# frobelbest/BANet

Hardware: NVIDIA H100
Metric: LM iters/sec (frame-pair LM iterations, 640x480x4-scale, K=128) (higher is better)
Workload: dtype tf32 level-wise (mma.sync tf32 x3 below 65536 points/pair, x1 above; f32 accumulate; everything else f32)

## Files before the change

### banet_b200/csrc/lm_build_tc6.cu

```cuda
#include "common.cuh"
#include "features.cuh"
#include "lm_build.h"
#include "tc_utils.cuh"
#include "mma_role.cuh"
#include "tmap.h"
#include <stdlib.h>

namespace banet { namespace v6 {
using namespace tc;

constexpr int TILE = 64, W0 = 4, GW = 8, AW = 4, MW = 4;
constexpr int THREADS = (W0 + GW + AW + MW) * 32;
constexpr int STAGE_A = 4 * TILE * 128, STAGE_R = 5 * TILE * 128;
constexpr int REC = 16;

template <int MODE, bool FLY, bool BB = false> struct Smem {
#ifndef BANET_TC6_NST1
#define BANET_TC6_NST1 4
#endif
#ifndef BANET_TC6_NST2
#define BANET_TC6_NST2 3
#endif
#ifndef BANET_TC6_NST3
#define BANET_TC6_NST3 2
#endif
#ifndef BANET_TC6_NREC
#define BANET_TC6_NREC 3
#endif
    static constexpr int NST = MODE == 1 ? BANET_TC6_NST1 : MODE == 2 ? BANET_TC6_NST2 : BANET_TC6_NST3;
    static constexpr int NREC = MODE == 3 ? 2 : BANET_TC6_NREC;
    static constexpr int STAGE = BB ? STAGE_A / 2 : STAGE_A;
    static constexpr int off_A = 0;
    static constexpr int off_R = NST * STAGE;
    static constexpr int off_Alo = off_R + STAGE_R;
    static constexpr int off_Rlo = off_Alo + (MODE >= 2 && !BB ? STAGE_A : 0);
    static constexpr int off_misc = off_Rlo + (MODE == 3 ? STAGE_R : 0);
    static constexpr int off_bar = off_misc;
    static constexpr int off_tile = off_misc + 192;
    static constexpr int off_pose = off_tile + 64;
    static constexpr int off_w = off_pose + W0 * 16 * 4;
    static constexpr int off_rec = off_w + W0 * 128 * 4;
    static constexpr int off_rbs = off_rec + NREC * TILE * REC * 4;
    static constexpr int off_ccs = off_rbs + GW * 128 * 4;
    static constexpr int total = off_ccs + AW * 28 * 4;
    static constexpr int slack = 1024;
    static constexpr int bytes = total + slack;
};

__device__ __forceinline__ long long gtime6() { long long t; asm volatile("mov.u64 %0, %%globaltimer;" : "=l"(t)); return t; }
#ifdef BANET_TC6_TRACE_ON
#define TC6_TRACE(role, it, slot) do { if (prm.trace && blockIdx.x == 1 && lane == 0 && (it) >= 16 && (it) < 48) \
        prm.trace[(((role) * 32 + ((it) - 16)) * 12) + (slot)] = gtime6(); } while (0)
#else
#define TC6_TRACE(role, it, slot) do { } while (0)
#endif
template <int NT> __device__ __forceinline__ void team_bar() { asm volatile("bar.sync 2, %0;" :: "n"(NT) : "memory"); }
__device__ __forceinline__ int reflect_i(int i, int n) { i = i < 0 ? -i : (i >= n ? 2 * n - 2 - i : i); return i < 0 ? 0 : i; }
__device__ __forceinline__ float4 ldg4(const float* p) { return __ldg(reinterpret_cast<const float4*>(p)); }
__device__ __forceinline__ float hsum16(float v) {
    v += __shfl_xor_sync(0xffffffffu, v, 8); v += __shfl_xor_sync(0xffffffffu, v, 4);
    v += __shfl_xor_sync(0xffffffffu, v, 2); v += __shfl_xor_sync(0xffffffffu, v, 1);
    return v;
}
struct TileCoord { int b, n0, cnt, tx0, ty0; };
__device__ __forceinline__ TileCoord tile_coord(const BuildParams& prm, long long tl) {
    TileCoord tc;
    const unsigned t = (unsigned)tl, tpp = (unsigned)prm.tiles_per_pair;
    tc.b = (int)(t / tpp);
    const int r = (int)(t - (unsigned)tc.b * tpp);
    if (prm.grid_w > 0) {
// ... 37 lines not shown
template <int NCH, bool FLY, int NREC>
__device__ __forceinline__ void gather_bf16(const BuildParams& prm, const int* sTile, float* sRec, float* sRbs, uint64_t* recs, uint64_t* gath,
                                            uint64_t* rbdump, uint64_t* rbfree, int ntiles, int g, int lane)
{
    constexpr int C = 64 * NCH, CPL = C / 16, PXW = TILE / GW;
    using TB = BfTap<CPL>;
    const int hw = lane >> 4, hl = lane & 15;
    const int N = prm.N, h = prm.h, w = prm.w, c2 = prm.c2;
    float rb[CPL];
#pragma unroll
    for (int u = 0; u < CPL; ++u) rb[u] = 0.f;
    typename TB::T tb[13];
    int cur_b = -1, ndump = 0;
    const uint64_t pol_stream = prm.l2_hints >= 1 ? l2_policy_evict_first() : l2_policy_evict_normal();
    const uint64_t pol_tap = prm.l2_hints >= 2 ? l2_policy_evict_last() : l2_policy_evict_normal();

    auto dump_rb = [&]() {
        if (ndump > 0) mbar_wait_parked(rbfree, (ndump - 1) & 1);
#pragma unroll
        for (int u = 0; u < CPL; ++u) rb[u] += __shfl_xor_sync(0xffffffffu, rb[u], 16);
        if (hw == 0) {
#pragma unroll
            for (int j = 0; j < CPL / 4; ++j)
                *reinterpret_cast<float4*>(sRbs + g * 128 + CPL * hl + 4 * j) = make_float4(rb[4 * j], rb[4 * j + 1], rb[4 * j + 2], rb[4 * j + 3]);
        }
        __syncwarp();
        if (lane == 0) mbar_arrive(rbdump);
#pragma unroll
        for (int u = 0; u < CPL; ++u) rb[u] = 0.f;
        ++ndump;
    };

    for (int j = 0; j < ntiles; ++j) {
        const int s = j % NREC;
        mbar_wait_parked(&recs[s], (j / NREC) & 1);
        const int b = sTile[s * 4];
        if (b != cur_b) { if (cur_b >= 0) dump_rb(); cur_b = b; }
        float* rec = sRec + (s * TILE + g * PXW) * REC;
        const bf16* c1b = static_cast<const bf16*>(prm.conv1) + (size_t)b * N * C + CPL * hl;
        const bf16* img = static_cast<const bf16*>(prm.conv2) + (size_t)b * h * w * c2 + CPL * hl;
#pragma unroll
        for (int u = 0; u < PXW / 2; ++u) {
            const int pl = 2 * u + hw;
            const float mask = rec[pl * REC + 4];
            float m11 = 0.f, m12 = 0.f, m22 = 0.f, q1 = 0.f, q2 = 0.f;
            if (mask != 0.f) {
                const uint4 o = *reinterpret_cast<const uint4*>(rec + pl * REC);
                const int n = __float_as_int(rec[pl * REC + 11]);
                auto ldt = [&](const bf16* q) { return TB::ld(q, pol_tap); };
                tb[0] = TB::ld_stream(c1b + (size_t)n * C, pol_stream);
// ... 34 lines not shown
                    q1 = fmaf(gx, d, q1); q2 = fmaf(gy, d, q2);
                    rb[i] += fabsf(d);
                }
            }
            m11 = hsum16(m11); m12 = hsum16(m12); m22 = hsum16(m22); q1 = hsum16(q1); q2 = hsum16(q2);
            if (hl == 0) {
                const float wn = (prm.weight && mask != 0.f) ? __ldg(prm.weight + (size_t)b * N + __float_as_int(rec[pl * REC + 11])) : 1.f;
                *reinterpret_cast<float4*>(rec + pl * REC + 12) = make_float4(m11 * wn, m12 * wn, m22 * wn, q1 * wn);
                rec[pl * REC + 11] = q2 * wn;
            }
        }
        __syncwarp();
        if (lane == 0) mbar_arrive(&gath[s]);
    }
    if (cur_b >= 0) dump_rb();
}

template <int NCH, bool FLY, int MODE, int KBLK = 4, typename TF = float, typename TB = float>
__global__ void __launch_bounds__(THREADS, 1)
lm_build_tc6_kernel(const __grid_constant__ CUtensorMap tmapB, const BuildParams prm)
{
    constexpr bool BB = sizeof(TB) == 2;
    using SM = Smem<MODE, FLY, BB>;
    constexpr int NST = SM::NST, NREC = SM::NREC;
    constexpr int BLK = BB ? 4096 : 8192;
    constexpr int KR = 32 * KBLK, EXTB = KBLK;
    extern __shared__ __align__(1024) unsigned char smem_raw[];
    unsigned char* base = smem_raw + ((1024u - (smem_u32(smem_raw) & 1023u)) & 1023u);
    uint64_t* bars = reinterpret_cast<uint64_t*>(base + SM::off_bar);
    uint64_t* fullB = bars;
// ... 24 lines not shown
        for (int i = 0; i < NREC; ++i) { mbar_init(&recs[i], W0); mbar_init(&gath[i], GW); mbar_init(&recfree[i], AW); }
        mbar_init(rfree, MW); mbar_init(rready, AW);
        mbar_init(rbdump, GW); mbar_init(rbfree, AW);
        fence_barrier_init();
        prefetch_tmap(&tmapB);
    }
    for (int i = tid; i < TILE * 8; i += THREADS) {
        const int r = i >> 3, c = i & 7;
        *reinterpret_cast<float4*>(base + SM::off_R + EXTB * 8192 + sw128_off(r, c)) = make_float4(0.f, 0.f, 0.f, 0.f);
        if (MODE == 3) *reinterpret_cast<float4*>(base + SM::off_Rlo + EXTB * 8192 + sw128_off(r, c)) = make_float4(0.f, 0.f, 0.f, 0.f);
    }
    __syncthreads();

    const int r16 = lane & 15, hf = lane >> 4;

    if (warp < W0) {
        setmaxnreg_dec<48>();
        const int gwi = warp, nlr = gwi * 16 + r16;
        float* myPose = sPose + gwi * 16;
        float* myW = sW + gwi * 128;
        int geom_b = -1;
        uint32_t dseed = 0;
        TileCoord nxt = tile_coord(prm, t_begin);
        int nxt_r = (int)((unsigned)t_begin - (unsigned)nxt.b * (unsigned)prm.tiles_per_pair);
        for (int j = 0; j < ntiles; ++j) {
            const TileCoord tc = nxt;
            if (++nxt_r == prm.tiles_per_pair) { nxt_r = 0; ++nxt.b; nxt.tx0 = 0; nxt.ty0 = 0; nxt.n0 = 0; nxt.cnt = grid2d ? TILE : min(TILE, N); }
            else if (grid2d && prm.band_rows > 1) nxt = tile_coord(prm, t_begin + j + 1);
            else if (grid2d) { nxt.tx0 += 8; if (nxt.tx0 >= prm.tiles_x * 8) { nxt.tx0 = 0; nxt.ty0 += 8; } }
            else { nxt.n0 += TILE; nxt.cnt = min(TILE, N - nxt.n0); }
            const int b = tc.b;
            if (gwi == 1 && j + 2 < ntiles) {
                const TileCoord tn = tile_coord(prm, t_begin + j + 2);
                if (grid2d) {
                    if (lane < 8) {
                        const int gy = tn.ty0 + lane;
                        if (gy < prm.grid_h && tn.tx0 < prm.grid_w) {
                            const size_t n = (size_t)gy * prm.grid_w + tn.tx0;
                            const int wpx = min(8, prm.grid_w - tn.tx0);
// ... 28 lines not shown
                    dseed = (__float_as_uint(__ldg(prm.W + (size_t)b * KR)) * 0x9E3779B1u) ^ (__float_as_uint(__ldg(prm.W + (size_t)b * KR + 1)) * 0x85EBCA77u)
                          ^ (__float_as_uint(__ldg(prm.W + (size_t)b * KR + 2)) * 0xC2B2AE3Du) ^ __float_as_uint(__ldg(prm.T + b * 3)) ^ (uint32_t)b;
                __syncwarp();
            }
            const int s = j % NST, sr = j % NREC;
            const unsigned char* As = base + SM::off_A + s * SM::STAGE;
            float p0 = 0.f, p1 = 0.f, p2 = 0.f, D0 = 0.f;
            int n = 0; bool valid = false;
            if (grid2d) { const int gx = tc.tx0 + (nlr & 7), gy = tc.ty0 + (nlr >> 3); valid = gx < prm.grid_w && gy < prm.grid_h; n = gy * prm.grid_w + gx; }
            else { valid = nlr < tc.cnt; n = tc.n0 + nlr; }
            if (lane < 16 && valid) {
                const float* pp = prm.p + (size_t)b * 3 * N + n;
                p0 = __ldg(pp); p1 = __ldg(pp + N); p2 = __ldg(pp + 2 * (size_t)N);
                D0 = __ldg(prm.D + (size_t)b * N + n);
            }
            if (gwi == 0) TC6_TRACE(2, j, 0);
            mbar_wait_parked(&recfree[sr], ((j / NREC) & 1) ^ 1);
            mbar_wait_parked(&fullB[s], (j / NST) & 1);
            if (gwi == 0) TC6_TRACE(2, j, 1);
            float mydot;
            {
                float4 acc = make_float4(0.f, 0.f, 0.f, 0.f);
                uint4 bq = make_uint4(0u, 0u, 0u, 0u);
#pragma unroll
                for (int i = 0; i < 16; ++i) {
                    const int blk = 2 * hf + (i >> 3), c = i & 7;
                    if (KBLK != 4 && blk >= KBLK) continue;
                    float4 bv;
                    if constexpr (BB) {
                        if ((c & 1) == 0) bq = *reinterpret_cast<const uint4*>(As + blk * BLK + sw64_off(nlr, c >> 1));
                        const uint32_t u0 = (c & 1) ? bq.z : bq.x, u1 = (c & 1) ? bq.w : bq.y;
                        bv = make_float4(bf16_lo(u0), bf16_hi(u0), bf16_lo(u1), bf16_hi(u1));
                    } else {
                        bv = *reinterpret_cast<const float4*>(As + blk * 8192 + sw128_off(nlr, c));
// ... 3 lines not shown
                    if constexpr (MODE == 1 && !BB) {
                        uint32_t hsh = dseed ^ ((uint32_t)n * 0x9E3779B1u) ^ ((uint32_t)(blk * 8 + c) * 0x85EBCA77u);
                        hsh ^= hsh >> 16; hsh *= 0x7FEB352Du; hsh ^= hsh >> 15;
                        uint32_t hs2 = hsh * 0x846CA68Bu; hs2 ^= hs2 >> 16;
                        *reinterpret_cast<float4*>(const_cast<unsigned char*>(As) + blk * 8192 + sw128_off(nlr, c)) =
                            make_float4(__uint_as_float((__float_as_uint(bv.x) + (hsh & 0x1fffu)) & 0xFFFFE000u),
                                        __uint_as_float((__float_as_uint(bv.y) + ((hsh >> 13) & 0x1fffu)) & 0xFFFFE000u),
                                        __uint_as_float((__float_as_uint(bv.z) + (hs2 & 0x1fffu)) & 0xFFFFE000u),
                                        __uint_as_float((__float_as_uint(bv.w) + ((hs2 >> 13) & 0x1fffu)) & 0xFFFFE000u));
                    }
                }
                if constexpr (MODE == 1 && !BB) fence_proxy_async_smem();
                mydot = (acc.x + acc.y) + (acc.z + acc.w);
                mydot += __shfl_xor_sync(0xffffffffu, mydot, 16);
            }
            if (gwi == 0) TC6_TRACE(2, j, 2);
            if (lane < 16) {
                const float* pose = myPose;
                float mask = 0.f, x = 0.f, y = 0.f, iZ = 0.f, rx = 0.f, ry = 0.f, rz = 0.f, dx = 0.f, dy = 0.f;
                int x0 = 0, y0 = 0;
                if (valid) {
                    const float Dt = D0 + mydot;
                    rx = pose[0] * p0 + pose[1] * p1 + pose[2] * p2;
                    ry = pose[3] * p0 + pose[4] * p1 + pose[5] * p2;
                    rz = pose[6] * p0 + pose[7] * p1 + pose[8] * p2;
                    const float X = rx * Dt + pose[9], Y = ry * Dt + pose[10], Z = rz * Dt + pose[11];
                    x = X / Z; y = Y / Z; iZ = 1.0f / Z;
                    const float u = pose[12] * x + pose[14], v = pose[13] * y + pose[15];
                    if ((u >= 0.f) && (u <= (float)(w - 1)) && (v >= 0.f) && (v <= (float)(h - 1)) && isfinite(iZ)) {
                        mask = 1.f;
                        const float fu = floorf(u), fv = floorf(v);
// ... 32 lines not shown
                        if (first_y && y0 > 0) prefetch_l2_bulk(imgp + ((size_t)(y0 - 1) * w + xs) * c2, by);
                        if (edge_y) {
                            if (y0 + 1 < h) prefetch_l2_bulk(imgp + ((size_t)(y0 + 1) * w + xs) * c2, by);
                            if (y0 + 2 < h) prefetch_l2_bulk(imgp + ((size_t)(y0 + 2) * w + xs) * c2, by);
                        }
                    }
                }
                float* rec = sRec + (sr * TILE + nlr) * REC;
                *reinterpret_cast<uint4*>(rec) = make_uint4(o[0], o[1], o[2], o[3]);
                *reinterpret_cast<float4*>(rec + 4) = make_float4(mask, x, y, iZ);
                *reinterpret_cast<float4*>(rec + 8) = make_float4(rx, ry, rz, __int_as_float(valid ? n : 0));
                *reinterpret_cast<float4*>(rec + 12) = make_float4(dx, dy, __uint_as_float(cx[0]), __uint_as_float(cx[1]));
            }
            if (gwi == 0 && lane == 0) sTile[sr * 4] = b;
            __syncwarp();
            if (gwi == 0) TC6_TRACE(2, j, 3);
            if (lane == 0) mbar_arrive(&recs[sr]);
        }
    } else if (warp < W0 + GW) {
        setmaxnreg_inc<112>();
        if constexpr (sizeof(TF) == 2) { gather_bf16<NCH, FLY, NREC>(prm, sTile, sRec, sRbs, recs, gath, rbdump, rbfree, ntiles, warp - W0, lane); return; }
        const int g = warp - W0, hw = lane >> 4, hl = lane & 15;
        constexpr int PXW = TILE / GW;
        constexpr int NUNIT = (PXW / 2) * NCH;
        float rb[NCH * 4];
#pragma unroll
        for (int u = 0; u < NCH * 4; ++u) rb[u] = 0.f;
        float4 tb[13];
        float m11 = 0.f, m12 = 0.f, m22 = 0.f, q1 = 0.f, q2 = 0.f;
        int cur_b = -1, ndump = 0;
        const uint64_t pol_stream = prm.l2_hints >= 1 ? l2_policy_evict_first() : l2_policy_evict_normal();
        const uint64_t pol_tap = prm.l2_hints >= 2 ? l2_policy_evict_last() : l2_policy_evict_normal();

        auto dump_rb = [&]() {
            if (ndump > 0) mbar_wait_parked(rbfree, (ndump - 1) & 1);
#pragma unroll
            for (int u = 0; u < NCH * 4; ++u) rb[u] += __shfl_xor_sync(0xffffffffu, rb[u], 16);
            if (hw == 0) {
#pragma unroll
                for (int j = 0; j < NCH; ++j)
                    *reinterpret_cast<float4*>(sRbs + g * 128 + 64 * j + 4 * hl) = make_float4(rb[4 * j], rb[4 * j + 1], rb[4 * j + 2], rb[4 * j + 3]);
            }
            __syncwarp();
            if (lane == 0) mbar_arrive(rbdump);
#pragma unroll
            for (int u = 0; u < NCH * 4; ++u) rb[u] = 0.f;
            ++ndump;
        };

        for (int j = 0; j < ntiles; ++j) {
            const int s = j % NREC;
            if (g == 0) TC6_TRACE(0, j, 0);
            mbar_wait_parked(&recs[s], (j / NREC) & 1);
            if (g == 0) TC6_TRACE(0, j, 1);
            const int b = sTile[s * 4];
            if (b != cur_b) { if (cur_b >= 0) dump_rb(); cur_b = b; }
            float* rec = sRec + (s * TILE + g * PXW) * REC;
            const float* c1b = static_cast<const float*>(prm.conv1) + (size_t)b * N * C + 4 * hl;
            const float* imgb = static_cast<const float*>(prm.conv2) + (size_t)b * h * w * c2 + 4 * hl;
#pragma unroll
            for (int u = 0; u < NUNIT; ++u) {
                const int pl = 2 * (u / NCH) + hw, co = 64 * (u % NCH), jc = u % NCH;
                const float mask = rec[pl * REC + 4];
                if (mask != 0.f) {
                    const uint4 o = *reinterpret_cast<const uint4*>(rec + pl * REC);
                    const int n = __float_as_int(rec[pl * REC + 11]);
                    const float* img = imgb + co;
                    auto ldt = [&](const float* q) { return ldg4_hint(q, pol_tap); };
                    tb[0] = ld_stream_f4_hint(c1b + (size_t)n * C + co, pol_stream);
// ... 46 lines not shown
                        }
                        BANET_CH(x, 0) BANET_CH(y, 1) BANET_CH(z, 2) BANET_CH(w, 3)
#undef BANET_CH
                    }
                }
                if (jc == NCH - 1) {
                    m11 = hsum16(m11); m12 = hsum16(m12); m22 = hsum16(m22); q1 = hsum16(q1); q2 = hsum16(q2);
                    if (hl == 0) {
                        const float wn = (prm.weight && mask != 0.f) ? __ldg(prm.weight + (size_t)b * N + __float_as_int(rec[pl * REC + 11])) : 1.f;
                        *reinterpret_cast<float4*>(rec + pl * REC + 12) = make_float4(m11 * wn, m12 * wn, m22 * wn, q1 * wn);
                        rec[pl * REC + 11] = q2 * wn;
                    }
                }
            }
            __syncwarp();
            if (g == 0) TC6_TRACE(0, j, 2);
            if (lane == 0) mbar_arrive(&gath[s]);
        }
        if (cur_b >= 0) dump_rb();
    } else if (warp < W0 + GW + AW) {
        setmaxnreg_dec<72>();
        const int awi = warp - (W0 + GW);
        const int atid = tid - (W0 + GW) * 32;
        const int nlr = awi * 16 + r16;
        const SlotLayout L{KR, C};
        unsigned char* Rs = base + SM::off_R;
        float cc[28];
#pragma unroll
        for (int q = 0; q < 28; ++q) cc[q] = 0.f;
        int scale_b = -1, sspan = -1;
        float fx = 0.f, fy = 0.f;
        int rr = (ntiles > 0) ? (int)((unsigned)t_begin % (unsigned)prm.tiles_per_pair) : 0;
        const uint64_t pol_basis = prm.l2_hints >= 1 ? l2_policy_evict_first() : l2_policy_evict_normal();
        auto issue_tma = [&](int t) {
            const int st = t % NST;
            const TileCoord tc = tile_coord(prm, t_begin + t);
            mbar_arrive_expect_tx(&fullB[st], KBLK * BLK);
            unsigned char* dst = base + SM::off_A + st * SM::STAGE;
            if (grid2d) {
#pragma unroll
                for (int blk = 0; blk < KBLK; ++blk) tma_load_3d_hint(dst + blk * BLK, &tmapB, blk * 32, tc.tx0, tc.b * prm.grid_h + tc.ty0, &fullB[st], pol_basis);
            } else {
                const int row = tc.b * N + tc.n0;
#pragma unroll
                for (int blk = 0; blk < KBLK; ++blk) tma_load_2d_hint(dst + blk * BLK, &tmapB, blk * 32, row, &fullB[st], pol_basis);
            }
        };
        auto flush = [&](int sp) {
            float* slot = prm.partials + ((size_t)blockIdx.x * prm.max_span + sp) * prm.slot_floats;
#pragma unroll
            for (int q = 0; q < 28; ++q) {
                float v = cc[q];
                v += __shfl_xor_sync(0xffffffffu, v, 8); v += __shfl_xor_sync(0xffffffffu, v, 4);
                v += __shfl_xor_sync(0xffffffffu, v, 2); v += __shfl_xor_sync(0xffffffffu, v, 1);
                if (lane == 0) sCcs[awi * 28 + q] = v;
                cc[q] = 0.f;
            }
            mbar_wait_parked(rbdump, sp & 1);
            team_bar<AW * 32>();
            if (atid < C) {
                float sum = 0.f;
#pragma unroll
                for (int wq = 0; wq < GW; ++wq) sum += sRbs[wq * 128 + atid];
                slot[L.off_rbar() + atid] = sum;
            }
            if (atid < 28) slot[L.off_cc() + atid] = (sCcs[atid] + sCcs[28 + atid]) + (sCcs[56 + atid] + sCcs[84 + atid]);
            team_bar<AW * 32>();
            if (lane == 0) mbar_arrive(rbfree);
        };

        if (awi == 0 && lane == 0)
            for (int t = 0; t < NST && t < ntiles; ++t) issue_tma(t);

        for (int j = 0; j < ntiles; ++j) {
            const int s = j % NST, sr = j % NREC;
            const bool last_of_pair = (++rr == prm.tiles_per_pair) || (j == ntiles - 1);
            if (rr == prm.tiles_per_pair) rr = 0;
            const unsigned char* As = base + SM::off_A + s * SM::STAGE;
            if (awi == 0) TC6_TRACE(1, j, 0);
            mbar_wait_parked(&gath[sr], (j / NREC) & 1);
            if (awi == 0) TC6_TRACE(1, j, 1);
            const int b = sTile[sr * 4];
            if (b != scale_b) { scale_b = b; ++sspan; fx = __ldg(prm.intr + b * 4); fy = __ldg(prm.intr + b * 4 + 1); }
            float ext[8] = {0.f, 0.f, 0.f, 0.f, 0.f, 0.f, 0.f, 0.f};
            if (lane < 16) {
                const float* rec = sRec + (sr * TILE + nlr) * REC;
                const float4 ra = *reinterpret_cast<const float4*>(rec + 12), rbq = *reinterpret_cast<const float4*>(rec + 4),
                             rc = *reinterpret_cast<const float4*>(rec + 8);
                if (rbq.x != 0.f) {
                    const float m11 = ra.x, m12 = ra.y, m22 = ra.z, q1 = ra.w, q2 = rc.w, x = rbq.y, y = rbq.z, iZ = rbq.w;
                    const float rx = rc.x, ry = rc.y, rz = rc.z;
                    const float a0[6] = {-fx * (x * y), -fx * (-1.f - x * x), -fx * y, -fx * (-iZ), 0.f, -fx * (x * iZ)};
                    const float a1[6] = {-fy * (1.f + y * y), -fy * (-(x * y)), -fy * (-x), 0.f, -fy * (-iZ), -fy * (y * iZ)};
                    float ux[6], uy[6];
#pragma unroll
                    for (int i = 0; i < 6; ++i) { ux[i] = m11 * a0[i] + m12 * a1[i]; uy[i] = m12 * a0[i] + m22 * a1[i]; }
// ... 4 lines not shown
                        for (int jj = i; jj < 6; ++jj) { cc[q] += a0[i] * ux[jj] + a1[i] * uy[jj]; ++q; }
#pragma unroll
                    for (int i = 0; i < 6; ++i) cc[21 + i] += a0[i] * q1 + a1[i] * q2;
                    cc[27] += 1.f;
                    const float jd0 = fx * ((rx - rz * x) * iZ), jd1 = fy * ((ry - rz * y) * iZ);
                    const float u0 = m11 * jd0 + m12 * jd1, u1 = m12 * jd0 + m22 * jd1;
#pragma unroll
                    for (int i = 0; i < 6; ++i) ext[i] = a0[i] * u0 + a1[i] * u1;
                    ext[6] = jd0 * q1 + jd1 * q2;
                    ext[7] = jd0 * u0 + jd1 * u1;
                }
            }
            __syncwarp();
            if (lane == 0) mbar_arrive(&recfree[sr]);
            const float sn = __shfl_sync(0xffffffffu, ext[7], r16);
            if (awi == 0) TC6_TRACE(1, j, 2);
            mbar_wait_parked(&fullB[s], (j / NST) & 1);
            if (j > 0) {
                mbar_wait_parked(rfree, (j - 1) & 1);
                if (awi == 0 && lane == 0 && j - 1 + NST < ntiles) issue_tma(j - 1 + NST);
            }
            if (awi == 0) TC6_TRACE(1, j, 3);
            if (lane < 16) {
                const float4 e0 = make_float4(tf32_rna(ext[0]), tf32_rna(ext[1]), tf32_rna(ext[2]), tf32_rna(ext[3]));
                const float4 e1 = make_float4(tf32_rna(ext[4]), tf32_rna(ext[5]), tf32_rna(ext[6]), 0.f);
                *reinterpret_cast<float4*>(Rs + EXTB * 8192 + sw128_off(nlr, 0)) = e0;
                *reinterpret_cast<float4*>(Rs + EXTB * 8192 + sw128_off(nlr, 1)) = e1;
                if constexpr (MODE == 3) {
                    *reinterpret_cast<float4*>(base + SM::off_Rlo + EXTB * 8192 + sw128_off(nlr, 0)) = make_float4(ext[0] - e0.x, ext[1] - e0.y, ext[2] - e0.z, ext[3] - e0.w);
                    *reinterpret_cast<float4*>(base + SM::off_Rlo + EXTB * 8192 + sw128_off(nlr, 1)) = make_float4(ext[4] - e1.x, ext[5] - e1.y, ext[6] - e1.z, 0.f);
                }
            }
            if constexpr (BB) {
#pragma unroll
                for (int i = 0; i < 8; ++i) {
                    const int blk = 2 * hf + (i >> 2), m = i & 3;
                    if (KBLK != 4 && blk >= KBLK) continue;
// ... 17 lines not shown
            for (int i = 0; i < 16; ++i) {
                if (KBLK != 4 && 2 * hf + (i >> 3) >= KBLK) continue;
                const uint32_t off = rowoff + (i >> 3) * 8192 + (((i & 7) + r16) & 7) * 16;
                const float4 bv = *reinterpret_cast<const float4*>(As + off);
                const float4 pv = make_float4(sn * bv.x, sn * bv.y, sn * bv.z, sn * bv.w);
                float4 hv;
                if constexpr (MODE == 3) hv = make_float4(tf32_rna(pv.x), tf32_rna(pv.y), tf32_rna(pv.z), tf32_rna(pv.w));
                else hv = make_float4(tf32_rna_bits(pv.x), tf32_rna_bits(pv.y), tf32_rna_bits(pv.z), tf32_rna_bits(pv.w));
                *reinterpret_cast<float4*>(Rs + off) = hv;
                if constexpr (MODE >= 2)
                    *reinterpret_cast<float4*>(base + SM::off_Alo + off) = make_float4(bv.x - tf32_trunc(bv.x), bv.y - tf32_trunc(bv.y), bv.z - tf32_trunc(bv.z), bv.w - tf32_trunc(bv.w));
                if constexpr (MODE == 3)
                    *reinterpret_cast<float4*>(base + SM::off_Rlo + off) = make_float4(pv.x - hv.x, pv.y - hv.y, pv.z - hv.z, pv.w - hv.w);
            }
            }
            if (awi == 0) TC6_TRACE(1, j, 4);
            __syncwarp();
            if (lane == 0) mbar_arrive(rready);
            if (awi == 0) TC6_TRACE(1, j, 5);
            if (last_of_pair) flush(sspan);
        }
    } else {
        setmaxnreg_inc<136>();
        mma_role<SM, SM::STAGE, MODE, KR, BB>(prm, base, fullB, rready, rfree, t_begin, ntiles, warp - (W0 + GW + AW), lane);
    }
}

template <int NCH, bool FLY, int MODE, int KBLK, typename TF, typename TB>
static int launch6(const CUtensorMap& tm, const BuildParams& prm, int grid, cudaStream_t st)
{
    auto kern = lm_build_tc6_kernel<NCH, FLY, MODE, KBLK, TF, TB>;
    const int smem = Smem<MODE, FLY, sizeof(TB) == 2>::bytes;
    cudaError_t e = cudaFuncSetAttribute(kern, cudaFuncAttributeMaxDynamicSharedMemorySize, smem);
    if (e != cudaSuccess) { set_error("lm_build_tc6: smem attr (%d B): %s", smem, cudaGetErrorString(e)); return BANET_ERR_CUDA; }
    kern<<<grid, THREADS, smem, st>>>(tm, prm);
    BANET_CUDA_LAUNCH_CHECK("lm_build_tc6_kernel launch");
    return BANET_OK;
}
template <int NCH, bool FLY, typename TF, typename TB>
// ... 29 lines not shown
```

### banet_b200/csrc/lm_build_tc_host.cu

```cuda
#include "common.cuh"
#include "lm_build.h"
#include "tc_utils.cuh"
#include "tmap.h"

namespace banet {

constexpr int TC_TILE = 64;

int lm_build_tc6_launch(int mode, bool fly, int nch, int kblk, bool is_bf16, bool basis_bf16, const CUtensorMap& tm, const BuildParams& prm, int grid,
                        cudaStream_t st);
int lm_build_tc7_launch(int mode, int nch, int kblk, const CUtensorMap& tmB, const CUtensorMap& tmF, const CUtensorMap& tmC, const BuildParams& prm, int grid,
                        cudaStream_t st);
bool lm_build_tc7_supported(int mode, int nch, int kblk);

constexpr int kTc6DefaultBandRows = 1, kTc6DefaultL2Hints = 0, kTc6DefaultTapPrefetch = 0;
static banet_tuning_t g_tuning = {0, 0, 4, 0, 0, 0};
void set_tuning(const banet_tuning_t& t) { g_tuning = t; }
const banet_tuning_t& tuning() { return g_tuning; }

static bool use_gen7(const banet_level_t* lv, int mode, int kblk)
{
    const bool wanted = g_tuning.tc_generation == 7;
    int wx = 0, wy = 0;
    lm_build_tc7_window(&wx, &wy);
    return wanted && !lv->weight && lv->feature_dtype == BANET_DTYPE_F32 && lv->basis_dtype == BANET_DTYPE_F32 && lv->conv2_channels == lv->C && lv->grid_w > 0 && lv->h < 65536 && lv->w < 65536 &&
           lv->h >= wy && lv->w >= wx && lm_build_tc7_supported(mode, lv->C / 64, kblk);
}

// ... 39 lines not shown
    if (lv->grid_w > 0) rc = make_tmap_basis_3d(&tm, lv->B, basis_bf16, (uint64_t)lv->nb * lv->grid_h, lv->grid_w, lv->K, 8, 8, 32);
    else rc = make_tmap_basis_2d(&tm, lv->B, basis_bf16, (uint64_t)lv->nb * lv->N, lv->K, TC_TILE, 32);
    if (rc) return rc;
    const bool fly = lv->conv2_channels == lv->C;
    BuildParams prm;
    prm.nb = lv->nb; prm.N = lv->N; prm.C = lv->C; prm.K = lv->K; prm.h = lv->h; prm.w = lv->w; prm.c2 = lv->conv2_channels;
    prm.conv1 = lv->conv1; prm.conv2 = lv->conv2; prm.intr = lv->intr; prm.p = lv->p; prm.D = lv->D; prm.B = lv->B;
    prm.R = R; prm.T = T; prm.W = W; prm.weight = lv->weight;
    prm.partials = reinterpret_cast<float*>(ws);
    prm.slot_floats = plan.slot_floats; prm.max_span = plan.max_span;
    prm.tiles_per_pair = plan.tiles_per_pair; prm.total_tiles = plan.total_tiles;
    prm.grid_w = lv->grid_w; prm.grid_h = lv->grid_h;
    prm.tiles_x = lv->grid_w > 0 ? (lv->grid_w + 7) / 8 : 0; prm.tiles_y = lv->grid_h > 0 ? (lv->grid_h + 7) / 8 : 0;
    prm.band_rows = 1; prm.l2_hints = 0; prm.tap_prefetch = 0; prm.kq_i = 0; prm.kq_j = 0;
    prm.hdd_transposed = 1;
    prm.trace = nullptr;
    const int nch = lv->C / 64;
    prm.force_direct = g_tuning.tc7_force_direct;
    if (use_gen7(lv, mode, kblk)) {
        int band = g_tuning.tc7_band_rows; if (band < 1) band = 1; if (band > prm.tiles_y) band = prm.tiles_y;
        prm.band_rows = band;
        CUtensorMap tmF;
        int wx = 0, wy = 0; lm_build_tc7_window(&wx, &wy);
        rc = make_tmap_f32_nhwc(&tmF, static_cast<const float*>(lv->conv2), lv->nb, lv->h, lv->w, lv->conv2_channels, 32, wx, wy);
        if (rc) return rc;
        CUtensorMap tmC;
        rc = make_tmap_f32_nhwc(&tmC, static_cast<const float*>(lv->conv1), lv->nb, lv->grid_h, lv->grid_w, lv->C, 32, 8, 8);
        if (rc) return rc;
        rc = lm_build_tc7_launch(mode, nch, kblk, tm, tmF, tmC, prm, plan.grid, st);
    } else {
        int band = g_tuning.tc6_band_rows > 0 ? g_tuning.tc6_band_rows : kTc6DefaultBandRows;
// ... 12 lines not shown
```

### banet_b200/csrc/mma_role.cuh

```cuda
#pragma once
#include "common.cuh"
#include "lm_build.h"
#include "tc_utils.cuh"

namespace banet { namespace tc {

__device__ __forceinline__ void mma_tf32_m16n8k8_z(float (&d)[4], const uint32_t (&a)[4], uint32_t b0, uint32_t b1) {
    asm("mma.sync.aligned.m16n8k8.row.col.f32.tf32.tf32.f32 {%0,%1,%2,%3}, {%4,%5,%6,%7}, {%8,%9}, {%10,%10,%10,%10};"
        : "=f"(d[0]), "=f"(d[1]), "=f"(d[2]), "=f"(d[3])
        : "r"(a[0]), "r"(a[1]), "r"(a[2]), "r"(a[3]), "r"(b0), "r"(b1), "f"(0.f));
}
__device__ __forceinline__ void mma_add_rn(float (&acc)[4], const uint32_t (&a)[4], uint32_t b0, uint32_t b1) {
    float p[4];
    mma_tf32_m16n8k8_z(p, a, b0, b1);
    acc[0] += p[0]; acc[1] += p[1]; acc[2] += p[2]; acc[3] += p[3];
}
__device__ __forceinline__ uint32_t tf32_bits(float x) { return __float_as_uint(x) & 0xFFFFE000u; }

__host__ __device__ constexpr int mma_full_groups(int mb) { return mb < 0 ? 0 : (mb + 1) / 2; }
__host__ __device__ constexpr bool mma_half_group(int mb) { return mb >= 0 && (mb & 1) == 0; }

template <int MB> struct MmaAcc {
    static constexpr int NF = mma_full_groups(MB);
    static constexpr bool HALF = mma_half_group(MB);
// ... 18 lines not shown
                for (int G = 0; G < NF; ++G)
#pragma unroll
                    for (int j = 0; j < 4; ++j) slot[(size_t)(32 * G + 16 * (e & 1) + 4 * t + j) * KR + i] = h[G][j][e];
                if constexpr (HALF) {
#pragma unroll
                    for (int j = 0; j < 2; ++j) slot[(size_t)(32 * NF + 2 * (e & 1) + 4 * t + j) * KR + i] = hh[j][e];
                }
                const int n = 2 * t + (e & 1);
                if (n < 7) slot[KR * KR + n * KR + i] = x[e];
            }
        }
        zero();
    }
};

template <class SM, int STAGE_A, int MODE, int KR, int MB0, int MB1, bool BB>
__device__ __forceinline__ void mma_warp(const BuildParams& prm, const unsigned char* base, uint64_t* fullB, uint64_t* rready,
                                         uint64_t* rfree, long long t_begin, int ntiles, int lane)
{
    constexpr int NST = SM::NST, EXTB = KR / 32;
    constexpr int NG0 = mma_full_groups(MB0), NG1 = mma_full_groups(MB1), NG = NG0 > NG1 ? NG0 : NG1;
    constexpr bool H0 = mma_half_group(MB0), H1 = mma_half_group(MB1);
    const int g = lane >> 2, t = lane & 3;
    const uint32_t oa = t * 128 + (((g >> 1) ^ t) << 4) + (g & 1) * 8;
    const uint32_t ob0 = t * 128 + ((((g >> 1) | ((g & 1) << 2)) ^ t) << 4);
    const uint32_t ob1 = (ob0 ^ 64) + 512;
    const uint32_t ox = EXTB * 8192 + t * 128 + (((g >> 2) ^ t) << 4) + (g & 3) * 4;
    const uint32_t oab = t * 64 + (((g >> 2) ^ (t >> 1)) << 4) + (g & 3) * 4;
    MmaAcc<MB0> acc0;
    MmaAcc<MB1> acc1;
    acc0.zero(); acc1.zero();
    int span = 0;
    int rr = (ntiles > 0) ? (int)((unsigned)t_begin % (unsigned)prm.tiles_per_pair) : 0;
    for (int j = 0; j < ntiles; ++j) {
        const int s = j % NST;
        mbar_wait_parked(rready, j & 1);
        mbar_wait_parked(&fullB[s], (j / NST) & 1);
        const unsigned char* ahi = base + SM::off_A + s * STAGE_A;
#pragma unroll 1
        for (int pass = 0; pass < MODE; ++pass) {
            if constexpr (BB) { if (pass == 1) continue; }
            const unsigned char* a = pass == 1 ? base + SM::off_Alo : ahi;
            const unsigned char* r = base + (pass == 2 ? SM::off_Rlo : SM::off_R);
#pragma unroll 1
            for (int kk = 0; kk < 8; ++kk) {
                const unsigned char* ak = a + kk * (BB ? 512 : 1024);
                const unsigned char* rk = BB ? r + kk * 1024 : ak + (r - a);
                uint32_t f0[4], f1[4];
                if constexpr (BB) {
                    if constexpr (MB0 >= 0) {
                        const uint32_t lo = *reinterpret_cast<const uint32_t*>(ak + (MB0 >> 1) * 4096 + oab + 32 * (MB0 & 1));
                        const uint32_t hi = *reinterpret_cast<const uint32_t*>(ak + (MB0 >> 1) * 4096 + 256 + oab + 32 * ((MB0 & 1) ^ 1));
// ... 37 lines not shown
                    for (int jb = 0; jb < 2; ++jb) {
                        if constexpr (H0) mma_add_rn(acc0.hh[jb], f0, b0[jb], b1[jb]);
                        else mma_add_rn(acc1.hh[jb], f1, b0[jb], b1[jb]);
                    }
                }
                if constexpr (MB0 >= 0) {
                    const uint32_t x0 = tf32_bits(*reinterpret_cast<const float*>(rk + ox));
                    const uint32_t x1 = tf32_bits(*reinterpret_cast<const float*>(rk + ox + 576));
                    mma_add_rn(acc0.x, f0, x0, x1);
                    if constexpr (MB1 >= 0) mma_add_rn(acc1.x, f1, x0, x1);
                }
            }
        }
        __syncwarp();
        if (lane == 0) mbar_arrive(rfree);
        const bool last_of_pair = (++rr == prm.tiles_per_pair) || (j == ntiles - 1);
        if (rr == prm.tiles_per_pair) rr = 0;
        if (last_of_pair) {
            float* slot = prm.partials + ((size_t)blockIdx.x * prm.max_span + span) * prm.slot_floats;
            acc0.template write<KR>(slot, g, t);
            acc1.template write<KR>(slot, g, t);
            ++span;
        }
    }
}

template <class SM, int STAGE_A, int MODE, int KR, bool BB = false>
__device__ __forceinline__ void mma_role(const BuildParams& prm, const unsigned char* base, uint64_t* fullB, uint64_t* rready,
                                         uint64_t* rfree, long long t_begin, int ntiles, int mw, int lane)
{
    constexpr int NMB = KR / 16;
#define BANET_MMA_WARP(A, B) mma_warp<SM, STAGE_A, MODE, KR, A, B, BB>(prm, base, fullB, rready, rfree, t_begin, ntiles, lane)
    if constexpr (NMB == 8) {
        switch (mw) { case 0: BANET_MMA_WARP(0, 7); break; case 1: BANET_MMA_WARP(1, 6); break;
                      case 2: BANET_MMA_WARP(2, 5); break; default: BANET_MMA_WARP(3, 4); break; }
    } else if constexpr (NMB == 4) {
        switch (mw) { case 0: BANET_MMA_WARP(0, -1); break; case 1: BANET_MMA_WARP(1, -1); break;
                      case 2: BANET_MMA_WARP(2, -1); break; default: BANET_MMA_WARP(3, -1); break; }
    } else {
        static_assert(NMB == 2, "K = 128, 64 or 32");
        switch (mw) { case 0: BANET_MMA_WARP(0, -1); break; case 1: BANET_MMA_WARP(1, -1); break; default: BANET_MMA_WARP(-1, -1); break; }
    }
#undef BANET_MMA_WARP
}

}}
```

### banet_b200/csrc/tc_utils.cuh

```cuda
#pragma once
#include <cuda.h>
#include <cuda_runtime.h>
#include <stdint.h>

namespace banet { namespace tc {

__device__ __forceinline__ uint32_t smem_u32(const void* p) { return (uint32_t)__cvta_generic_to_shared(p); }

__device__ __forceinline__ void mbar_init(uint64_t* bar, uint32_t count) {
    asm volatile("mbarrier.init.shared::cta.b64 [%0], %1;" :: "r"(smem_u32(bar)), "r"(count) : "memory");
}
__device__ __forceinline__ void fence_barrier_init() {
    asm volatile("fence.mbarrier_init.release.cluster;" ::: "memory");
}
__device__ __forceinline__ void mbar_arrive(uint64_t* bar) {
    asm volatile("{\n\t.reg .b64 st;\n\tmbarrier.arrive.shared::cta.b64 st, [%0];\n\t}" :: "r"(smem_u32(bar)) : "memory");
}
__device__ __forceinline__ void mbar_arrive_expect_tx(uint64_t* bar, uint32_t bytes) {
    asm volatile("{\n\t.reg .b64 st;\n\tmbarrier.arrive.expect_tx.shared::cta.b64 st, [%0], %1;\n\t}"
                 :: "r"(smem_u32(bar)), "r"(bytes) : "memory");
}
__device__ __forceinline__ bool mbar_try_wait(uint64_t* bar, uint32_t parity) {
    uint32_t ok;
    asm volatile("{\n\t.reg .pred p;\n\tmbarrier.try_wait.parity.shared::cta.b64 p, [%1], %2;\n\tselp.b32 %0, 1, 0, p;\n\t}"
                 : "=r"(ok) : "r"(smem_u32(bar)), "r"(parity) : "memory");
    return ok != 0;
}
__device__ __forceinline__ void mbar_wait(uint64_t* bar, uint32_t parity) {
    while (!mbar_try_wait(bar, parity)) { }
}

__device__ __forceinline__ void mbar_wait_parked(uint64_t* bar, uint32_t parity) {
    asm volatile("{\n\t.reg .pred p;\n\tWAIT_%=:\n\tmbarrier.try_wait.parity.shared::cta.b64 p, [%0], %1, %2;\n\t@p bra DONE_%=;\n\tbra WAIT_%=;\n\tDONE_%=:\n\t}"
                 :: "r"(smem_u32(bar)), "r"(parity), "r"(0x989680) : "memory");
}
__device__ __forceinline__ void mbar_wait_sleep(uint64_t* bar, uint32_t parity) {
    while (!mbar_try_wait(bar, parity)) { __nanosleep(40); }
}
__device__ __forceinline__ bool mbar_wait_bounded(uint64_t* bar, uint32_t parity, int max_iters) {
    for (int i = 0; i < max_iters; ++i) { if (mbar_try_wait(bar, parity)) return true; __nanosleep(64); }
    return false;
}
template <int NREG> __device__ __forceinline__ void setmaxnreg_inc() { asm volatile("setmaxnreg.inc.sync.aligned.u32 %0;" :: "n"(NREG)); }
template <int NREG> __device__ __forceinline__ void setmaxnreg_dec() { asm volatile("setmaxnreg.dec.sync.aligned.u32 %0;" :: "n"(NREG)); }

__device__ __forceinline__ void fence_proxy_async_smem() { asm volatile("fence.proxy.async.shared::cta;" ::: "memory"); }

__device__ __forceinline__ void prefetch_tmap(const CUtensorMap* m) {
    asm volatile("prefetch.tensormap [%0];" :: "l"(reinterpret_cast<uint64_t>(m)) : "memory");
}
__device__ __forceinline__ void tma_load_2d(void* dst, const CUtensorMap* m, int c0, int c1, uint64_t* bar) {
    asm volatile("cp.async.bulk.tensor.2d.shared::cluster.global.mbarrier::complete_tx::bytes [%0], [%1, {%3, %4}], [%2];"
                 :: "r"(smem_u32(dst)), "l"(reinterpret_cast<uint64_t>(m)), "r"(smem_u32(bar)), "r"(c0), "r"(c1) : "memory");
// ... 86 lines not shown
```

Before: 7761.

## Move TMA basis refill into MMA warp and cut mode-1 stages to two

Moves issuing of the basis TMA loads from the algebra warps to the first MMA warp. That warp now refills a stage as soon as all MMA warps release it, instead of waiting for the algebra role to get there. Because refill happens earlier, the mode-1 stage count drops from 4 to 2, freeing shared memory. Also swaps the ad-hoc globaltimer trace for an optional per-role wait-cycle profiler that compiles to plain waits by default. Risks include MMA warp 0 stalling on rfree before continuing its own work, and less prefetch depth with only two stages.

```diff
diff --git a/banet_b200/csrc/lm_build_tc6.cu b/banet_b200/csrc/lm_build_tc6.cu
--- a/banet_b200/csrc/lm_build_tc6.cu
+++ b/banet_b200/csrc/lm_build_tc6.cu
@@ -16,7 +16,7 @@
 
 template <int MODE, bool FLY, bool BB = false> struct Smem {
 #ifndef BANET_TC6_NST1
-#define BANET_TC6_NST1 4
+#define BANET_TC6_NST1 2
 #endif
 #ifndef BANET_TC6_NST2
 #define BANET_TC6_NST2 3
@@ -47,13 +47,6 @@
     static constexpr int bytes = total + slack;
 };
 
-__device__ __forceinline__ long long gtime6() { long long t; asm volatile("mov.u64 %0, %%globaltimer;" : "=l"(t)); return t; }
-#ifdef BANET_TC6_TRACE_ON
-#define TC6_TRACE(role, it, slot) do { if (prm.trace && blockIdx.x == 1 && lane == 0 && (it) >= 16 && (it) < 48) \
-        prm.trace[(((role) * 32 + ((it) - 16)) * 12) + (slot)] = gtime6(); } while (0)
-#else
-#define TC6_TRACE(role, it, slot) do { } while (0)
-#endif
 template <int NT> __device__ __forceinline__ void team_bar() { asm volatile("bar.sync 2, %0;" :: "n"(NT) : "memory"); }
 __device__ __forceinline__ int reflect_i(int i, int n) { i = i < 0 ? -i : (i >= n ? 2 * n - 2 - i : i); return i < 0 ? 0 : i; }
 __device__ __forceinline__ float4 ldg4(const float* p) { return __ldg(reinterpret_cast<const float4*>(p)); }
@@ -121,9 +114,10 @@
     int cur_b = -1, ndump = 0;
     const uint64_t pol_stream = prm.l2_hints >= 1 ? l2_policy_evict_first() : l2_policy_evict_normal();
     const uint64_t pol_tap = prm.l2_hints >= 2 ? l2_policy_evict_last() : l2_policy_evict_normal();
+    ROLE_CLOCK_START();
 
     auto dump_rb = [&]() {
-        if (ndump > 0) mbar_wait_parked(rbfree, (ndump - 1) & 1);
+        if (ndump > 0) ROLE_WAIT(rbfree, (ndump - 1) & 1, WAIT_RBFREE);
 #pragma unroll
         for (int u = 0; u < CPL; ++u) rb[u] += __shfl_xor_sync(0xffffffffu, rb[u], 16);
         if (hw == 0) {
@@ -140,7 +134,7 @@
 
     for (int j = 0; j < ntiles; ++j) {
         const int s = j % NREC;
-        mbar_wait_parked(&recs[s], (j / NREC) & 1);
+        ROLE_WAIT(&recs[s], (j / NREC) & 1, WAIT_RECS);
         const int b = sTile[s * 4];
         if (b != cur_b) { if (cur_b >= 0) dump_rb(); cur_b = b; }
         float* rec = sRec + (s * TILE + g * PXW) * REC;
@@ -205,6 +199,7 @@
         if (lane == 0) mbar_arrive(&gath[s]);
     }
     if (cur_b >= 0) dump_rb();
+    ROLE_FINISH(ROLE_GATHER, ntiles);
 }
 
 template <int NCH, bool FLY, int MODE, int KBLK = 4, typename TF = float, typename TB = float>
@@ -259,6 +254,21 @@
 
     const int r16 = lane & 15, hf = lane >> 4;
 
+    auto issue_tma = [&](int t, int st) {
+        const uint64_t pol_basis = prm.l2_hints >= 1 ? l2_policy_evict_first() : l2_policy_evict_normal();
+        const TileCoord tc = tile_coord(prm, t_begin + t);
+        mbar_arrive_expect_tx(&fullB[st], KBLK * BLK);
+        unsigned char* dst = base + SM::off_A + st * SM::STAGE;
+        if (grid2d) {
+#pragma unroll
+            for (int blk = 0; blk < KBLK; ++blk) tma_load_3d_hint(dst + blk * BLK, &tmapB, blk * 32, tc.tx0, tc.b * prm.grid_h + tc.ty0, &fullB[st], pol_basis);
+        } else {
+            const int row = tc.b * N + tc.n0;
+#pragma unroll
+            for (int blk = 0; blk < KBLK; ++blk) tma_load_2d_hint(dst + blk * BLK, &tmapB, blk * 32, row, &fullB[st], pol_basis);
+        }
+    };
+
     if (warp < W0) {
         setmaxnreg_dec<48>();
         const int gwi = warp, nlr = gwi * 16 + r16;
@@ -268,6 +278,7 @@
         uint32_t dseed = 0;
         TileCoord nxt = tile_coord(prm, t_begin);
         int nxt_r = (int)((unsigned)t_begin - (unsigned)nxt.b * (unsigned)prm.tiles_per_pair);
+        ROLE_CLOCK_START();
         for (int j = 0; j < ntiles; ++j) {
             const TileCoord tc = nxt;
             if (++nxt_r == prm.tiles_per_pair) { nxt_r = 0; ++nxt.b; nxt.tx0 = 0; nxt.ty0 = 0; nxt.n0 = 0; nxt.cnt = grid2d ? TILE : min(TILE, N); }
@@ -326,10 +337,8 @@
                 p0 = __ldg(pp); p1 = __ldg(pp + N); p2 = __ldg(pp + 2 * (size_t)N);
                 D0 = __ldg(prm.D + (size_t)b * N + n);
             }
-            if (gwi == 0) TC6_TRACE(2, j, 0);
-            mbar_wait_parked(&recfree[sr], ((j / NREC) & 1) ^ 1);
-            mbar_wait_parked(&fullB[s], (j / NST) & 1);
-            if (gwi == 0) TC6_TRACE(2, j, 1);
+            ROLE_WAIT(&recfree[sr], ((j / NREC) & 1) ^ 1, WAIT_RECFREE);
+            ROLE_WAIT(&fullB[s], (j / NST) & 1, WAIT_FULLB);
             float mydot;
             {
                 float4 acc = make_float4(0.f, 0.f, 0.f, 0.f);
@@ -363,7 +372,6 @@
                 mydot = (acc.x + acc.y) + (acc.z + acc.w);
                 mydot += __shfl_xor_sync(0xffffffffu, mydot, 16);
             }
-            if (gwi == 0) TC6_TRACE(2, j, 2);
             if (lane < 16) {
                 const float* pose = myPose;
                 float mask = 0.f, x = 0.f, y = 0.f, iZ = 0.f, rx = 0.f, ry = 0.f, rz = 0.f, dx = 0.f, dy = 0.f;
@@ -426,9 +434,9 @@
             }
             if (gwi == 0 && lane == 0) sTile[sr * 4] = b;
             __syncwarp();
-            if (gwi == 0) TC6_TRACE(2, j, 3);
             if (lane == 0) mbar_arrive(&recs[sr]);
         }
+        ROLE_FINISH(ROLE_GEOMETRY, ntiles);
     } else if (warp < W0 + GW) {
         setmaxnreg_inc<112>();
         if constexpr (sizeof(TF) == 2) { gather_bf16<NCH, FLY, NREC>(prm, sTile, sRec, sRbs, recs, gath, rbdump, rbfree, ntiles, warp - W0, lane); return; }
@@ -443,9 +451,10 @@
         int cur_b = -1, ndump = 0;
         const uint64_t pol_stream = prm.l2_hints >= 1 ? l2_policy_evict_first() : l2_policy_evict_normal();
         const uint64_t pol_tap = prm.l2_hints >= 2 ? l2_policy_evict_last() : l2_policy_evict_normal();
+        ROLE_CLOCK_START();
 
         auto dump_rb = [&]() {
-            if (ndump > 0) mbar_wait_parked(rbfree, (ndump - 1) & 1);
+            if (ndump > 0) ROLE_WAIT(rbfree, (ndump - 1) & 1, WAIT_RBFREE);
 #pragma unroll
             for (int u = 0; u < NCH * 4; ++u) rb[u] += __shfl_xor_sync(0xffffffffu, rb[u], 16);
             if (hw == 0) {
@@ -462,9 +471,7 @@
 
         for (int j = 0; j < ntiles; ++j) {
             const int s = j % NREC;
-            if (g == 0) TC6_TRACE(0, j, 0);
-            mbar_wait_parked(&recs[s], (j / NREC) & 1);
-            if (g == 0) TC6_TRACE(0, j, 1);
+            ROLE_WAIT(&recs[s], (j / NREC) & 1, WAIT_RECS);
             const int b = sTile[s * 4];
             if (b != cur_b) { if (cur_b >= 0) dump_rb(); cur_b = b; }
             float* rec = sRec + (s * TILE + g * PXW) * REC;
@@ -541,10 +548,10 @@
                 }
             }
             __syncwarp();
-            if (g == 0) TC6_TRACE(0, j, 2);
             if (lane == 0) mbar_arrive(&gath[s]);
         }
         if (cur_b >= 0) dump_rb();
+        ROLE_FINISH(ROLE_GATHER, ntiles);
     } else if (warp < W0 + GW + AW) {
         setmaxnreg_dec<72>();
         const int awi = warp - (W0 + GW);
@@ -558,21 +565,7 @@
         int scale_b = -1, sspan = -1;
         float fx = 0.f, fy = 0.f;
         int rr = (ntiles > 0) ? (int)((unsigned)t_begin % (unsigned)prm.tiles_per_pair) : 0;
-        const uint64_t pol_basis = prm.l2_hints >= 1 ? l2_policy_evict_first() : l2_policy_evict_normal();
-        auto issue_tma = [&](int t) {
-            const int st = t % NST;
-            const TileCoord tc = tile_coord(prm, t_begin + t);
-            mbar_arrive_expect_tx(&fullB[st], KBLK * BLK);
-            unsigned char* dst = base + SM::off_A + st * SM::STAGE;
-            if (grid2d) {
-#pragma unroll
-                for (int blk = 0; blk < KBLK; ++blk) tma_load_3d_hint(dst + blk * BLK, &tmapB, blk * 32, tc.tx0, tc.b * prm.grid_h + tc.ty0, &fullB[st], pol_basis);
-            } else {
-                const int row = tc.b * N + tc.n0;
-#pragma unroll
-                for (int blk = 0; blk < KBLK; ++blk) tma_load_2d_hint(dst + blk * BLK, &tmapB, blk * 32, row, &fullB[st], pol_basis);
-            }
-        };
+        ROLE_CLOCK_START();
         auto flush = [&](int sp) {
             float* slot = prm.partials + ((size_t)blockIdx.x * prm.max_span + sp) * prm.slot_floats;
 #pragma unroll
@@ -583,7 +576,7 @@
                 if (lane == 0) sCcs[awi * 28 + q] = v;
                 cc[q] = 0.f;
             }
-            mbar_wait_parked(rbdump, sp & 1);
+            ROLE_WAIT(rbdump, sp & 1, WAIT_RBDUMP);
             team_bar<AW * 32>();
             if (atid < C) {
                 float sum = 0.f;
@@ -595,18 +588,13 @@
             team_bar<AW * 32>();
             if (lane == 0) mbar_arrive(rbfree);
         };
-
-        if (awi == 0 && lane == 0)
-            for (int t = 0; t < NST && t < ntiles; ++t) issue_tma(t);
 
         for (int j = 0; j < ntiles; ++j) {
             const int s = j % NST, sr = j % NREC;
             const bool last_of_pair = (++rr == prm.tiles_per_pair) || (j == ntiles - 1);
             if (rr == prm.tiles_per_pair) rr = 0;
             const unsigned char* As = base + SM::off_A + s * SM::STAGE;
-            if (awi == 0) TC6_TRACE(1, j, 0);
-            mbar_wait_parked(&gath[sr], (j / NREC) & 1);
-            if (awi == 0) TC6_TRACE(1, j, 1);
+            ROLE_WAIT(&gath[sr], (j / NREC) & 1, WAIT_GATH);
             const int b = sTile[sr * 4];
             if (b != scale_b) { scale_b = b; ++sspan; fx = __ldg(prm.intr + b * 4); fy = __ldg(prm.intr + b * 4 + 1); }
             float ext[8] = {0.f, 0.f, 0.f, 0.f, 0.f, 0.f, 0.f, 0.f};
@@ -641,13 +629,8 @@
             __syncwarp();
             if (lane == 0) mbar_arrive(&recfree[sr]);
             const float sn = __shfl_sync(0xffffffffu, ext[7], r16);
-            if (awi == 0) TC6_TRACE(1, j, 2);
-            mbar_wait_parked(&fullB[s], (j / NST) & 1);
-            if (j > 0) {
-                mbar_wait_parked(rfree, (j - 1) & 1);
-                if (awi == 0 && lane == 0 && j - 1 + NST < ntiles) issue_tma(j - 1 + NST);
-            }
-            if (awi == 0) TC6_TRACE(1, j, 3);
+            ROLE_WAIT(&fullB[s], (j / NST) & 1, WAIT_FULLB);
+            if (j > 0) ROLE_WAIT(rfree, (j - 1) & 1, WAIT_RFREE);
             if (lane < 16) {
                 const float4 e0 = make_float4(tf32_rna(ext[0]), tf32_rna(ext[1]), tf32_rna(ext[2]), tf32_rna(ext[3]));
                 const float4 e1 = make_float4(tf32_rna(ext[4]), tf32_rna(ext[5]), tf32_rna(ext[6]), 0.f);
@@ -695,15 +678,17 @@
                     *reinterpret_cast<float4*>(base + SM::off_Rlo + off) = make_float4(pv.x - hv.x, pv.y - hv.y, pv.z - hv.z, pv.w - hv.w);
             }
             }
-            if (awi == 0) TC6_TRACE(1, j, 4);
             __syncwarp();
             if (lane == 0) mbar_arrive(rready);
-            if (awi == 0) TC6_TRACE(1, j, 5);
             if (last_of_pair) flush(sspan);
         }
+        ROLE_FINISH(ROLE_ALGEBRA, ntiles);
     } else {
         setmaxnreg_inc<136>();
-        mma_role<SM, SM::STAGE, MODE, KR, BB>(prm, base, fullB, rready, rfree, t_begin, ntiles, warp - (W0 + GW + AW), lane);
+        const int mw = warp - (W0 + GW + AW);
+        if (mw == 0 && lane == 0)
+            for (int t = 0; t < NST && t < ntiles; ++t) issue_tma(t, t);
+        mma_role<SM, SM::STAGE, MODE, KR, BB>(prm, base, fullB, rready, rfree, t_begin, ntiles, mw, lane, issue_tma);
     }
 }
 
diff --git a/banet_b200/csrc/lm_build_tc_host.cu b/banet_b200/csrc/lm_build_tc_host.cu
--- a/banet_b200/csrc/lm_build_tc_host.cu
+++ b/banet_b200/csrc/lm_build_tc_host.cu
@@ -12,6 +12,24 @@
 int lm_build_tc7_launch(int mode, int nch, int kblk, const CUtensorMap& tmB, const CUtensorMap& tmF, const CUtensorMap& tmC, const BuildParams& prm, int grid,
                         cudaStream_t st);
 bool lm_build_tc7_supported(int mode, int nch, int kblk);
+
+#ifdef BANET_TC6_ROLES
+static long long* g_roles = nullptr;
+constexpr int kRolesSlots = tc::NUM_ROLES * tc::ROLE_SLOTS;
+static long long* roles_buffer()
+{
+    if (!g_roles && cudaMalloc(&g_roles, kRolesSlots * sizeof(long long)) == cudaSuccess)
+        cudaMemset(g_roles, 0, kRolesSlots * sizeof(long long));
+    return g_roles;
+}
+extern "C" int banet_tc6_roles_take(long long* out, int n)
+{
+    if (!roles_buffer() || n < kRolesSlots) return BANET_ERR_CUDA;
+    if (cudaDeviceSynchronize() != cudaSuccess || cudaMemcpy(out, g_roles, kRolesSlots * sizeof(long long), cudaMemcpyDeviceToHost) != cudaSuccess ||
+        cudaMemset(g_roles, 0, kRolesSlots * sizeof(long long)) != cudaSuccess) return BANET_ERR_CUDA;
+    return kRolesSlots;
+}
+#endif
 
 constexpr int kTc6DefaultBandRows = 1, kTc6DefaultL2Hints = 0, kTc6DefaultTapPrefetch = 0;
 static banet_tuning_t g_tuning = {0, 0, 4, 0, 0, 0};
@@ -81,7 +99,11 @@
     prm.tiles_x = lv->grid_w > 0 ? (lv->grid_w + 7) / 8 : 0; prm.tiles_y = lv->grid_h > 0 ? (lv->grid_h + 7) / 8 : 0;
     prm.band_rows = 1; prm.l2_hints = 0; prm.tap_prefetch = 0; prm.kq_i = 0; prm.kq_j = 0;
     prm.hdd_transposed = 1;
+#ifdef BANET_TC6_ROLES
+    prm.trace = roles_buffer();
+#else
     prm.trace = nullptr;
+#endif
     const int nch = lv->C / 64;
     prm.force_direct = g_tuning.tc7_force_direct;
     if (use_gen7(lv, mode, kblk)) {
diff --git a/banet_b200/csrc/mma_role.cuh b/banet_b200/csrc/mma_role.cuh
--- a/banet_b200/csrc/mma_role.cuh
+++ b/banet_b200/csrc/mma_role.cuh
@@ -1,4 +1,5 @@
 #pragma once
+#include <type_traits>
 #include "common.cuh"
 #include "lm_build.h"
 #include "tc_utils.cuh"
@@ -56,10 +57,13 @@
     }
 };
 
-template <class SM, int STAGE_A, int MODE, int KR, int MB0, int MB1, bool BB>
+struct NoRefill { __device__ __forceinline__ void operator()(int, int) const {} };
+
+template <class SM, int STAGE_A, int MODE, int KR, int MB0, int MB1, bool BB, class Refill>
 __device__ __forceinline__ void mma_warp(const BuildParams& prm, const unsigned char* base, uint64_t* fullB, uint64_t* rready,
-                                         uint64_t* rfree, long long t_begin, int ntiles, int lane)
+                                         uint64_t* rfree, long long t_begin, int ntiles, int lane, const Refill& refill)
 {
+    constexpr bool REFILL = !std::is_same<Refill, NoRefill>::value;
     constexpr int NST = SM::NST, EXTB = KR / 32;
     constexpr int NG0 = mma_full_groups(MB0), NG1 = mma_full_groups(MB1), NG = NG0 > NG1 ? NG0 : NG1;
     constexpr bool H0 = mma_half_group(MB0), H1 = mma_half_group(MB1);
@@ -74,10 +78,11 @@
     acc0.zero(); acc1.zero();
     int span = 0;
     int rr = (ntiles > 0) ? (int)((unsigned)t_begin % (unsigned)prm.tiles_per_pair) : 0;
+    int s = 0, sph = 0;
+    ROLE_CLOCK_START();
     for (int j = 0; j < ntiles; ++j) {
-        const int s = j % NST;
-        mbar_wait_parked(rready, j & 1);
-        mbar_wait_parked(&fullB[s], (j / NST) & 1);
+        ROLE_WAIT(rready, j & 1, WAIT_RREADY);
+        ROLE_WAIT(&fullB[s], sph, WAIT_FULLB);
         const unsigned char* ahi = base + SM::off_A + s * STAGE_A;
 #pragma unroll 1
         for (int pass = 0; pass < MODE; ++pass) {
@@ -145,6 +150,13 @@
         }
         __syncwarp();
         if (lane == 0) mbar_arrive(rfree);
+        if constexpr (REFILL && MB0 == 0) {
+            if (lane == 0 && j + NST < ntiles) {
+                ROLE_WAIT(rfree, j & 1, WAIT_RFREE);
+                refill(j + NST, s);
+            }
+        }
+        if (++s == NST) { s = 0; sph ^= 1; }
         const bool last_of_pair = (++rr == prm.tiles_per_pair) || (j == ntiles - 1);
         if (rr == prm.tiles_per_pair) rr = 0;
         if (last_of_pair) {
@@ -154,14 +166,15 @@
             ++span;
         }
     }
+    ROLE_FINISH(ROLE_MMA, ntiles);
 }
 
-template <class SM, int STAGE_A, int MODE, int KR, bool BB = false>
+template <class SM, int STAGE_A, int MODE, int KR, bool BB = false, class Refill = NoRefill>
 __device__ __forceinline__ void mma_role(const BuildParams& prm, const unsigned char* base, uint64_t* fullB, uint64_t* rready,
-                                         uint64_t* rfree, long long t_begin, int ntiles, int mw, int lane)
+                                         uint64_t* rfree, long long t_begin, int ntiles, int mw, int lane, const Refill& refill = Refill())
 {
     constexpr int NMB = KR / 16;
-#define BANET_MMA_WARP(A, B) mma_warp<SM, STAGE_A, MODE, KR, A, B, BB>(prm, base, fullB, rready, rfree, t_begin, ntiles, lane)
+#define BANET_MMA_WARP(A, B) mma_warp<SM, STAGE_A, MODE, KR, A, B, BB, Refill>(prm, base, fullB, rready, rfree, t_begin, ntiles, lane, refill)
     if constexpr (NMB == 8) {
         switch (mw) { case 0: BANET_MMA_WARP(0, 7); break; case 1: BANET_MMA_WARP(1, 6); break;
                       case 2: BANET_MMA_WARP(2, 5); break; default: BANET_MMA_WARP(3, 4); break; }
diff --git a/banet_b200/csrc/tc_utils.cuh b/banet_b200/csrc/tc_utils.cuh
--- a/banet_b200/csrc/tc_utils.cuh
+++ b/banet_b200/csrc/tc_utils.cuh
@@ -37,6 +37,40 @@
 __device__ __forceinline__ void mbar_wait_sleep(uint64_t* bar, uint32_t parity) {
     while (!mbar_try_wait(bar, parity)) { __nanosleep(40); }
 }
+enum RoleId { ROLE_GEOMETRY, ROLE_GATHER, ROLE_ALGEBRA, ROLE_MMA, NUM_ROLES };
+enum WaitId { WAIT_FULLB, WAIT_RECS, WAIT_GATH, WAIT_RECFREE, WAIT_RREADY, WAIT_RFREE, WAIT_RBDUMP, WAIT_RBFREE, NUM_WAITS };
+constexpr int ROLE_SLOTS = 3 + NUM_WAITS;
+#ifdef BANET_TC6_ROLES
+struct RoleClock {
+    long long t0, w[NUM_WAITS];
+    __device__ __forceinline__ void start() {
+        t0 = clock64();
+#pragma unroll
+        for (int i = 0; i < NUM_WAITS; ++i) w[i] = 0;
+    }
+    __device__ __forceinline__ void wait(uint64_t* bar, uint32_t parity, int kind) {
+        const long long a = clock64();
+        mbar_wait_parked(bar, parity);
+        w[kind] += clock64() - a;
+    }
+    __device__ __forceinline__ void finish(long long* trace, int role, int ntiles, int lane) {
+        const long long run = clock64() - t0;
+        if (trace == nullptr || lane != 0) return;
+        unsigned long long* t = reinterpret_cast<unsigned long long*>(trace) + role * ROLE_SLOTS;
+        atomicAdd(t, (unsigned long long)run); atomicAdd(t + 1, 1ull); atomicAdd(t + 2, (unsigned long long)ntiles);
+#pragma unroll
+        for (int i = 0; i < NUM_WAITS; ++i) atomicAdd(t + 3 + i, (unsigned long long)w[i]);
+    }
+};
+#define ROLE_CLOCK_START() RoleClock clk; clk.start()
+#define ROLE_WAIT(bar, parity, kind) clk.wait(bar, parity, kind)
+#define ROLE_FINISH(role, ntiles) clk.finish(prm.trace, role, ntiles, lane)
+#else
+#define ROLE_CLOCK_START() do { } while (0)
+#define ROLE_WAIT(bar, parity, kind) mbar_wait_parked(bar, parity)
+#define ROLE_FINISH(role, ntiles) do { } while (0)
+#endif
+
 __device__ __forceinline__ bool mbar_wait_bounded(uint64_t* bar, uint32_t parity, int max_iters) {
     for (int i = 0; i < max_iters; ++i) { if (mbar_try_wait(bar, parity)) return true; __nanosleep(64); }
     return false;
```

Measured after the change: 7799 (median of 6 runs). About the same (+0.5%).
